# HKUST-Aerial-Robotics/VINS-Mono

Measured on AMD Instinct MI355X. Metric: sliding-window BA solves/sec (Estimator::optimization: 8-iteration dogleg solve + marginalization), higher is better.
Workload: dtype f64; 1 GPU; batch of 256 independent EuRoC-shape windows per step and GPU (K=11 frames, ~150 landmarks, 10 IMU factors, ~600 projection factors, 75-dim marginalization prior, max 8 iterations, MARGIN_OLD marginalization); windows resident in HBM; consecutive steps are issued to 16 HIP streams (independent batches in flight); windows_per_gpu=256, batches_in_flight=16, parallelism=independent batches x1 (no collectives)

## Files before the change

vins-mono_amd/csrc/ba_host.hip:

```cpp
#include "vg_range.h"
#include <hip/hip_runtime.h>
#include <algorithm>
#include <chrono>
#include <cmath>
#include <cstdio>
#include <cstdlib>
#include <cstring>
#include <string>
#include <thread>
#include <vector>
#include "ba_layout.h"
#include "vg_handle.h"
#include "../../include/vinsgpu.h"

struct BaFork { hipStream_t aux; hipEvent_t fork, join; };
extern "C" hipError_t ba_launch_solve(const BaLayout& L, const BaLayout* dL, const BaPtrs& P, int rounds, hipStream_t stream,
                                      hipEvent_t* ev, int* kinds, int* n_launches, const BaFork* fk);
typedef int (*BaAllReduce)(void* user, double* buf, size_t count, void* stream);
extern "C" hipError_t ba_launch_solve_big(const BaLayout& L, const BaLayout* dL, const BaPtrs& P, int rounds, int slack, hipStream_t stream,
                                          BaAllReduce allreduce, void* user, int* hook_rc, hipEvent_t* ev, int* kinds, int* n_launches);
extern "C" hipError_t ba_launch_eval_factors(const BaLayout& L, const BaLayout* dL, const BaPtrs& P, double* proj_r, double* proj_J,
                                            double* imu_r, double* imu_J, double* prior_r, hipStream_t stream);
extern "C" const char* ba_failed_launch();
extern "C" hipError_t ba_prepare_launch();
// ... 252 lines not shown
            if (L.lds_solve_w8 > 160 * 1024) L.sv_w8 = 0;
        }
    }
    if (L.big) {
        const int nt = (L.Rc + 1 + 15) / 16;
        L.nts = nt * (nt + 1) / 2;
        const int ntri = L.Rc * (L.Rc + 1) / 2;
        L.rb1_T = up(ntri + L.Rc, 2);
        L.rb1_scal = L.rb1_T + up((L.Rc + 1) * (L.Rc + 2) / 2, 2);
        L.rb1_len = L.rb1_scal + RB1_NSCAL;
    }
    int o = 0;
    L.io_hdr = o; o += BA_HDR_INTS;
    L.io_lm_start = o; o += L.Lcap;
    L.io_lm_fbeg = o; o += L.Lcap + 8;
    L.io_fac_i = o; o += L.Fcap;
    L.io_fac_j = o; o += L.Fcap;
    L.io_fac_lm = o; o += L.Fcap;
    L.io_fac_oi = o; o += L.Fcap;
    L.io_fac_oj = o; o += L.Fcap;
    L.io_fac_slot = o; o += L.Fcap;
    L.io_pair_ptr = o; o += up(L.Kp * L.Kp + 1, 8);
    L.io_task_list = o; o += up(L.ntask, 8);
    L.io_imu_valid = o; o += up(L.K, 8);
    L.io_pb_kind = o; o += L.NBcap;
    L.io_pb_idx = o; o += L.NBcap;
    L.io_pb_col = o; o += L.NBcap;
    L.io_pb_off = o; o += L.NBcap;
    L.io_pb_x0off = o; o += L.NBcap;
    L.istride = up(o, 8);
    o = 0;
    L.do_pose = o; o += up(7 * L.Kp, 2);
    L.do_sb = o; o += up(9 * L.K, 2);
    L.do_ex = o; o += 8;
    L.do_td = o; o += 2;
    L.do_lam = o; o += L.Lcap;
    L.do_obs = o; o += L.Ocap * BA_OBS_STRIDE;
    L.do_imu = o; o += (L.K - 1) * BA_IMU_STRIDE;
    L.do_par = o; o += P_NPAR;
    L.dstride = up(o, 8);
    L.pld = std::max(up(6 * L.K + 9 * 2 + 6 + 1, 8), L.Ncap);
    L.po_x0 = 0;
    L.po_r0 = 9 * std::max(up(L.K + 4, 8), L.NBcap);
    L.po_J0 = L.po_r0 + L.pld;
    L.pstride = up(L.po_J0 + L.pld * L.pld, 8);
    o = 0;
    L.so_ctl = o; o += C_NCTL;
    L.so_part = o; o += up(L.nbl, 8);
    L.so_x = o; o += 2 * L.nst;
    L.so_lam = o; o += 2 * L.Lcap;
    L.so_imuU = o; o += up((L.K - 1) * 225, 2);
    L.so_Hp = o; o += L.Ncap * L.Ncap;
    L.so_J0t = o; o += L.Ncap * L.Ncap;
    L.so_rec = o; o += L.Fcap * L.REC;
    L.so_sc = o; o += L.Rpad;
    L.so_sl = o; o += L.Lcap;
    L.so_dg = o; o += L.Rpad + L.Lcap;
    L.so_gt = o; o += L.Rpad + L.Lcap;
    L.so_gn = o; o += L.Rpad + L.Lcap;
    L.so_yl = o; o += L.Lcap;
    L.so_lsc = o; o += L.Lcap;
    L.so_xp = 0;
    if (!L.big) { L.so_xp = o; o += up(9 * L.K, 4) * L.ldc; }
    if (L.big) {
        L.so_bigm = o; o += up(bigm_doubles, 8);
        L.so_dgl = o; o += 2 * L.Lcap;
        L.so_gtl = o; o += 2 * L.Lcap;
    }
    {
        int b = 0;
        L.bo_Sp = b; b += up(L.Rc * (L.Rc + 1) / 2, 2);
        L.bo_gp = b; b += L.RcPad;
        L.bo_h = b; b += L.Lcap;
        L.bo_b = b; b += L.Lcap;
        L.bo_Wt = b; b += L.RcPad * L.Lcap;
        L.bo_imuJ = b; b += (L.K - 1) * 512;
        L.bo_pr = b; b += L.Ncap;
        L.bo_gpr = b; b += L.Ncap;
        L.buf_stride = up(b, 8);
    }
    L.so_buf = o; o += 2 * L.buf_stride;
    L.sstride = up(o, 8);
    L.pl_off = (int)((sizeof(BaLayout) + 255) / 256 * 256);
    L.pl_n = L.big ? 0 : L.Rc * (L.Rc + 1) / 2 + L.Rpad + 2 * 81 * L.K;
    o = 0;
    L.oo_pose = o; o += up(7 * L.Kp, 2);
    L.oo_sb = o; o += up(9 * L.K, 2);
    L.oo_ex = o; o += 8;
    L.oo_td = o; o += 2;
    L.oo_lam = o; o += L.Lcap;
    L.oo_sum = o; o += BA_SUM_DOUBLES;
    L.oo_trace = o; o += 5 * VG_MAX_ITERS + 16;
    L.ostride = up(o, 8);
    L.oi_stride = up(4 + VG_MAX_ITERS, 8);
    L.mcap = up(6 * L.K + 9 * 2 + 6 + 1, 8);
    if (L.mcap > 256) { h->err = "kept dimension of the marginalization beyond the kernel's tables"; return VG_ERR_UNSUPPORTED; }
    const int mcap = L.mcap;
    L.mo_J0 = 0;
    L.mo_r0 = mcap * mcap;
    L.mo_x0 = L.mo_r0 + mcap;
    L.mo_stride = up(L.mo_x0 + (L.K + 4) * 9, 8);
    L.mi_stride = up(8 + 2 * (L.K + 4) + 16, 8);
    L.mg_posmax = up(mcap + 15 + L.Lcap, 2);
    {
        const int nstm = up(16 * L.K + 8 + 1, 2);
        L.mg_cs = up(std::max(std::max(2 * mcap, 3 * (L.mg_posmax / 2 + 2)), 2 * (3 * ((mcap + 2) / 2) + 2) + 2), 2);
        L.mg_cs = std::max(L.mg_cs, std::max(up(5 * mcap + 8, 2), up(L.Lcap + 512, 2)));
// ... 1412 lines not shown
```

vins-mono_amd/csrc/ba_pipeline.hip:

```cpp
#include <hip/hip_runtime.h>
#include <vector>
#include <mutex>
#include <cstring>
#include <cstdlib>
#include "ba_layout.h"
#include "ba_factors.h"
#include "../../include/vinsgpu.h"

extern __shared__ __attribute__((aligned(16))) char bp_smem[];

#ifdef BA_SOLVE_W8_TU
#undef BA_PROFILE_DETAIL
#undef BA_DEBUG_DUMP
namespace vg_w8 {
#endif

#define NOINL __device__ __noinline__
#define AS_LDS(p) ((lds_d*)(p))
#define AS_LDS_C(p) ((const lds_d*)(p))
#define AS_GLB(p) ((glb_d*)(p))
#define AS_GLB_C(p) ((const glb_d*)(p))
#define AS_GLB_CI(p) ((const glb_i*)(p))
template <bool BIG> struct MovT { typedef lds_d D; typedef lds_i I; };
template <> struct MovT<true> { typedef glb_d D; typedef glb_i I; };
// ... 274 lines not shown
            for (int r = 0; r < 15; ++r) Uo[r * 15 + i] = (i >= r) ? A[i * 15 + r] : 0.0;
        __syncthreads();
    }
}

NOINL void imu_sqrt_info(const Ctx& c_in, int fbeg, int fend) {
    const Ctx c = c_in;
    const BaLayout L = *c.Lp;
    lds_d* A = AS_LDS(LDSB + c.wave * 256);
    const int nimu = fend < L.K - 1 ? fend : L.K - 1;
    const glb_i* valid = AS_GLB_CI(c.ia + L.io_imu_valid);
    const int li = c.lane < 15 ? c.lane : 14;
    for (int base = fbeg; base < nimu; base += BA_NW) {
        const int f = uni(base + c.wave);
        if (!(f < nimu && valid[f])) continue;
        const glb_d* cov = AS_GLB_C(c.di + L.do_imu + f * BA_IMU_STRIDE + IM_COV);
        double a[15];
#pragma unroll
        for (int k = 0; k < 15; ++k) a[k] = cov[li * 15 + k];
#pragma unroll
        for (int j = 14; j >= 0; --j) {
            const double d = sqrt(readlane_f64(a[j], j));
            a[j] = c.lane < j ? a[j] / d : (c.lane == j ? d : a[j]);
#pragma unroll
            for (int kk = 0; kk < j; ++kk) {
                const double ukj = readlane_f64(a[j], kk);
                a[kk] = (c.lane <= kk) ? a[kk] - a[j] * ukj : a[kk];
            }
        }
        if (c.lane < 15) {
#pragma unroll
            for (int k = 0; k < 15; ++k) A[c.lane * 15 + k] = a[k];
        }
        __builtin_amdgcn_wave_barrier();
        glb_d* Uo = AS_GLB(c.sc + L.so_imuU + f * 225);
        if (c.lane < 15) {
            const int j = c.lane;
            double x[15];
#pragma unroll
            for (int i = 14; i >= 0; --i) {
                double s = (i == j) ? 1.0 : 0.0;
#pragma unroll
                for (int k = 14; k > i; --k) s -= (k <= j) ? A[i * 15 + k] * x[k] : 0.0;
                x[i] = (i <= j) ? s / A[i * 15 + i] : 0.0;
            }
#pragma unroll
            for (int i = 0; i < 15; ++i) Uo[i * 15 + j] = x[i];
        }
        __builtin_amdgcn_wave_barrier();
    }
    __syncthreads();
}

#ifndef BA_SOLVE_W8_TU
extern "C" __global__ __launch_bounds__(BA_NT) void ba_prologue_kernel(const BaLayout* __restrict__ Lp, BaPtrs P) {
    const BaLayout& L = *Lp;
    Ctx c;
    ctx_init(c, Lp, P, blockIdx.x);
    double* x = c.sc + L.so_x;
    DP_DECL;
    const bool all = gridDim.y == 1;
    const int part = blockIdx.y, nI = (L.K - 1 + BA_NW - 1) / BA_NW;
    if (all || part == 0)
    {
        double* out = P.out + (size_t)blockIdx.x * L.ostride;
        int* iout = P.iout + (size_t)blockIdx.x * L.oi_stride;
        int* miout = P.miout + (size_t)blockIdx.x * L.mi_stride;
        for (int k = c.tid; k < L.ostride; k += BA_NT) out[k] = 0.0;
        for (int k = c.tid; k < L.oi_stride; k += BA_NT) iout[k] = 0;
        for (int k = c.tid; k < L.mi_stride; k += BA_NT) miout[k] = 0;
    }
    if (all || part == 0) {
        for (int k = c.tid; k < 7 * L.Kp; k += BA_NT) x[k] = c.di[L.do_pose + k];
        for (int k = c.tid; k < 9 * L.K; k += BA_NT) x[7 * L.Kp + k] = c.di[L.do_sb + k];
        if (c.tid < 7) x[7 * L.Kp + 9 * L.K + c.tid] = c.di[L.do_ex + c.tid];
        if (c.tid == 7) x[7 * L.Kp + 9 * L.K + 7] = c.di[L.do_td];
        for (int k = c.tid; k < c.nL; k += BA_NT) c.sc[L.so_lam + k] = c.di[L.do_lam + k];
        if (c.tid < C_NCTL) {
            double v = 0.0;
            if (c.tid == C_RADIUS) v = 1e4;
            if (c.tid == C_MU || c.tid == C_MUSOLVED) v = 1e-8;
            if (c.tid == C_T0) v = (double)wall_clock64();
            c.sc[L.so_ctl + c.tid] = v;
        }
    }
    DP_ADD(40);
    if (all || (part >= 1 && part <= nI)) {
        const int fbeg = all ? 0 : (part - 1) * BA_NW, fend = all ? L.K - 1 : part * BA_NW;
        if (L.imu_info) imu_sqrt_info_ref(c, fbeg, fend);
        else imu_sqrt_info(c, fbeg, fend);
    }
    DP_ADD(41);
    if (c.nprior && (all || part > nI)) {
        const bool do_copy = all || part == nI + 1, do_prod = all || part == nI + 2;
        const int n = c.nprior;
        const double* J0 = c.pri + L.po_J0;
        double* Hp = c.sc + L.so_Hp;
        if (do_copy) {
            double* J0t = c.sc + L.so_J0t;
            for (int wk = c.tid; wk < n * n; wk += BA_NT) { const int r = wk / n, cc = wk % n; J0t[cc * L.Ncap + r] = J0[r * L.pld + cc]; }
        }
        __syncthreads();
        DP_ADD(42);
        if (!do_prod) {
        } else if ((size_t)n * n * 8 <= (size_t)L.lds_pro) {
            double* J0s = LDSB;
            for (int wk = c.tid; wk < n * n; wk += BA_NT) J0s[wk] = J0[(wk / n) * L.pld + wk % n];
            __syncthreads();
            DP_ADD(43);
            const int T = (n + 15) >> 4, ntile = T * (T + 1) / 2, nks = (n + 3) >> 2;
            const int wave = c.tid >> 6, lane = c.tid & 63, li = lane & 15, lk = lane >> 4;
            for (int t = wave; t < ntile; t += BA_NT / 64) {
                int ta, tb;
                tri_decode(t, ta, tb);
                const int ca = 16 * ta + li, cb = 16 * tb + li;
                double4_t acc = (double4_t){0, 0, 0, 0};
                for (int ks = 0; ks < nks; ++ks) {
                    const int r = 4 * ks + lk;
                    const double av = (r < n && ca < n) ? J0s[r * n + ca] : 0.0;
                    const double bv = (r < n && cb < n) ? J0s[r * n + cb] : 0.0;
                    acc = __builtin_amdgcn_mfma_f64_16x16x4f64(av, bv, acc, 0, 0, 0);
                }
#pragma unroll
                for (int q = 0; q < 4; ++q) {
                    const int a = 16 * ta + lk + 4 * q, bb = 16 * tb + li;
                    if (a < n && bb <= a) {
                        Hp[a * L.Ncap + bb] = acc[q];
                    }
                }
            }
        } else {
            const int ld = L.pld;
            for (int wk = c.tid; wk < n * (n + 1) / 2; wk += BA_NT) {
                int a, bb;
                tri_decode(wk, a, bb);
                double s0 = 0.0, s1 = 0.0;
                int r = 0;
                for (; r + 1 < n; r += 2) { s0 += J0[r * ld + a] * J0[r * ld + bb]; s1 += J0[(r + 1) * ld + a] * J0[(r + 1) * ld + bb]; }
                if (r < n) s0 += J0[r * ld + a] * J0[r * ld + bb];
// ... 230 lines not shown
    double cost = 0.0;
    for (int w = c.tid; w < 4 * L.Ncap; w += BA_NT) {
        const int r = w % L.Ncap, q = w / L.Ncap;
        double sacc = 0.0;
        if (r < n)
            for (int k = q; k < n; k += 4) sacc += Jl[r * ld + k] * dx[k];
        part[w] = sacc;
    }
    __syncthreads();
    lds_d* rl = dx;
    double rv = 0.0;
    const bool own = c.tid < n;
    if (own) rv = r0[c.tid] + ((part[c.tid] + part[L.Ncap + c.tid]) + (part[2 * L.Ncap + c.tid] + part[3 * L.Ncap + c.tid]));
    __syncthreads();
    if (own) { pr[c.tid] = rv; rl[c.tid] = rv; cost += rv * rv; }
    __syncthreads();
    for (int w = c.tid; w < 4 * L.Ncap; w += BA_NT) {
        const int a = w % L.Ncap, q = w / L.Ncap;
        double sacc = 0.0;
        if (a < n)
            for (int k = q; k < n; k += 4) sacc += Jl[k * ld + a] * rl[k];
        part[w] = sacc;
    }
    __syncthreads();
    for (int a = c.tid; a < n; a += BA_NT)
        gpr[a] = (part[a] + part[L.Ncap + a]) + (part[2 * L.Ncap + a] + part[3 * L.Ncap + a]);
    __syncthreads();
    return cost;
}

struct ProjIn {
    double pi[7], pj[7], oi[8], oj[8], ex[8];
    double lam;
    int i, j, l;
};
DEV void proj_fetch(const Ctx& c, int f, const double* x_, const double* lam_, ProjIn& p) {
    const BaLayout& L = *c.Lp;
    const glb_i* ia = AS_GLB_CI(c.ia);
    const glb_d* x = AS_GLB_C(x_);
    const glb_d* obs = AS_GLB_C(c.di + L.do_obs);
    p.i = ia[L.io_fac_i + f];
    p.j = ia[L.io_fac_j + f];
    p.l = ia[L.io_fac_lm + f];
    const int oi = ia[L.io_fac_oi + f], oj = ia[L.io_fac_oj + f];
#pragma unroll
    for (int k = 0; k < 7; ++k) { p.pi[k] = x[7 * p.i + k]; p.pj[k] = x[7 * p.j + k]; }
#pragma unroll
    for (int k = 0; k < 8; ++k) {
        p.oi[k] = obs[oi * BA_OBS_STRIDE + k];
        p.oj[k] = obs[oj * BA_OBS_STRIDE + k];
        p.ex[k] = x[7 * L.Kp + 9 * L.K + k];
    }
    p.lam = AS_GLB_C(lam_)[p.l];
}
DEV void proj_fetch_staged(const Ctx& c, int f, const lds_d* xs, const double* lam_, ProjIn& p) {
    const BaLayout& L = *c.Lp;
    const glb_i* ia = AS_GLB_CI(c.ia);
    const glb_d* obs = AS_GLB_C(c.di + L.do_obs);
    p.i = ia[L.io_fac_i + f];
    p.j = ia[L.io_fac_j + f];
    p.l = ia[L.io_fac_lm + f];
    const int oi = ia[L.io_fac_oi + f], oj = ia[L.io_fac_oj + f];
#pragma unroll
    for (int k = 0; k < 8; ++k) {
        p.oi[k] = obs[oi * BA_OBS_STRIDE + k];
        p.oj[k] = obs[oj * BA_OBS_STRIDE + k];
    }
    p.lam = AS_GLB_C(lam_)[p.l];
#pragma unroll
    for (int k = 0; k < 7; ++k) { p.pi[k] = xs[7 * p.i + k]; p.pj[k] = xs[7 * p.j + k]; }
#pragma unroll
    for (int k = 0; k < 8; ++k) p.ex[k] = xs[7 * L.Kp + 9 * L.K + k];
}
DEV void proj_jac(const Ctx& c, const ProjIn& p, double* r, double* Ji, double* Jj, double* Jex,
                  double* Jl, double* Jtd) {
    const BaLayout& L = *c.Lp;
    if (L.t) {
        if (L.e) proj_eval<true, true, true>(p.pi, p.pj, p.ex, p.lam, p.oi, p.oj, p.ex[7], c.focal, c.tr, c.row, r, Ji, Jj, Jex, Jl, Jtd);
        else proj_eval<true, true, false>(p.pi, p.pj, p.ex, p.lam, p.oi, p.oj, p.ex[7], c.focal, c.tr, c.row, r, Ji, Jj, Jex, Jl, Jtd);
    } else {
        if (L.e) proj_eval<false, true, true>(p.pi, p.pj, p.ex, p.lam, p.oi, p.oj, 0.0, c.focal, c.tr, c.row, r, Ji, Jj, Jex, Jl, Jtd);
        else proj_eval<false, true, false>(p.pi, p.pj, p.ex, p.lam, p.oi, p.oj, 0.0, c.focal, c.tr, c.row, r, Ji, Jj, Jex, Jl, Jtd);
    }
}

NOINL double proj_linearize(const Ctx& c_in, int f, const double* x, const double* lam, double* recs) {
    const Ctx c = c_in;
    const BaLayout L = *c.Lp;
    ProjIn p;
    proj_fetch(c, f, x, lam, p);
    double r[2], Ji[12], Jj[12], Jex[12], Jl[2], Jtd[2];
    proj_jac(c, p, r, Ji, Jj, Jex, Jl, Jtd);
    const double s = r[0] * r[0] + r[1] * r[1];
    const double sq = sqrt(1.0 / (1.0 + s));
    glb_d* rec = AS_GLB(recs) + (size_t)AS_GLB_CI(c.ia)[L.io_fac_slot + f] * L.REC;
#pragma unroll
    for (int k = 0; k < 6; ++k) {
        rec[2 * k] = sq * Ji[k]; rec[2 * k + 1] = sq * Ji[6 + k];
        rec[12 + 2 * k] = sq * Jj[k]; rec[12 + 2 * k + 1] = sq * Jj[6 + k];
    }
    rec[24] = sq * Jl[0]; rec[25] = sq * Jl[1];
    rec[26] = sq * r[0]; rec[27] = sq * r[1];
    if (L.e) {
#pragma unroll
        for (int k = 0; k < 6; ++k) { rec[28 + 2 * k] = sq * Jex[k]; rec[28 + 2 * k + 1] = sq * Jex[6 + k]; }
    }
    if (L.t) { rec[28 + 12 * L.e] = sq * Jtd[0]; rec[29 + 12 * L.e] = sq * Jtd[1]; }
    return log1p(s);
}
NOINL double proj_cost(const Ctx& c_in, int f, const double* x, const double* lam) {
    const Ctx c = c_in;
    const BaLayout L = *c.Lp;
    ProjIn p;
    proj_fetch(c, f, x, lam, p);
    double r[2];
    if (L.t) proj_eval<true, false, false>(p.pi, p.pj, p.ex, p.lam, p.oi, p.oj, p.ex[7], c.focal, c.tr, c.row, r, 0, 0, 0, 0, 0);
    else proj_eval<false, false, false>(p.pi, p.pj, p.ex, p.lam, p.oi, p.oj, 0.0, c.focal, c.tr, c.row, r, 0, 0, 0, 0, 0);
    return log1p(r[0] * r[0] + r[1] * r[1]);
}

#ifndef BA_PROJ_WAVES
#define BA_PROJ_WAVES 1
#endif
#ifndef BA_SOLVE_W8_TU
extern "C" __global__ __launch_bounds__(BA_LIN_NT, BA_PROJ_WAVES) void ba_linearize_proj_kernel(const BaLayout* __restrict__ Lp, BaPtrs P, int cost_only) {
// ... 200 lines not shown
    buf[L.bo_b + l] = b;
    int row = 6 * L.Kp;
    if (L.e | L.t) {
        double wex[6] = {0, 0, 0, 0, 0, 0}, wtd = 0.0;
        const int otd = 28 + 12 * L.e;
        for (int f = fb; f < fe; ++f) {
            const double* rec = recs + (size_t)c.ia[L.io_fac_slot + f] * REC;
            const double l0 = rec[24], l1 = rec[25];
            if (L.e) {
#pragma unroll
                for (int k = 0; k < 6; ++k) wex[k] += rec[28 + 2 * k] * l0 + rec[28 + 2 * k + 1] * l1;
            }
            if (L.t) wtd += rec[otd] * l0 + rec[otd + 1] * l1;
        }
        if (L.e) {
#pragma unroll
            for (int k = 0; k < 6; ++k) Wt[(size_t)(col_ex(L) + k) * ldw] = anchor >= 0 ? wex[k] : 0.0;
            row += 6;
        }
        if (L.t) { Wt[(size_t)col_td(L) * ldw] = anchor >= 0 ? wtd : 0.0; row += 1; }
    }
    if (L.big) { Wt[row * ldw] = b; ++row; }
    for (; row < L.RcPad; ++row) Wt[row * ldw] = 0.0;
}

#ifndef BA_SOLVE_W8_TU
extern "C" __global__ __launch_bounds__(BA_ACC_NT) void ba_accumulate_kernel(const BaLayout* __restrict__ Lp, BaPtrs P) {
    const BaLayout& L = *Lp;
    const int bid = blockIdx.x;
    const int xcd = bid & 7, rest = bid >> 3;
    const int bx = rest % L.nba, w = (rest / L.nba) * 8 + xcd;
    if (w >= L.nwin) return;
    Ctx c;
    ctx_init(c, Lp, P, w);
    const double* ctl = c.sc + L.so_ctl;
    if (ctl[C_DONE] != 0.0) return;
    const int which = ((int)ctl[C_CUR]) ^ (ctl[C_PENDING] != 0.0 ? 1 : 0);
    double* buf = lin_buf(c, which);
    const double* recs = c.sc + L.so_rec;
    __shared__ double part[7 * 36 + 4];
    if (bx < L.Kp) { diag_pose_task(c, bx, recs, buf + L.bo_Sp, buf + L.bo_gp, part); return; }
    const int ng = L.e + L.t;
    if (ng && bx == L.Kp) { global_task(c, recs, buf + L.bo_Sp, buf + L.bo_gp, part); return; }
    const int g = (bx - L.Kp - (ng ? 1 : 0)) * (BA_ACC_NT / 64) + c.wave;
    const int nother = L.ntask - L.Kp - ng * (ng + 1) / 2;
    if (g < nother) owner_task(c, c.ia[L.io_task_list + g], c.lane, recs, buf + L.bo_Sp, buf + L.bo_gp);
    else {
        const int l = (g - nother) * 64 + c.lane;
        if (l < L.Lcap) landmark_task(c, l, recs, buf);
    }
}
#endif

#define LA_NT BA_NT
#define LA_RS 33
#define LA_NPW 6
#define LA_MAXP 13
#define LA_QCAP 80
static_assert(LA_QCAP <= 128, "the pair prefix of ba_linacc_proj_kernel takes two pairs per lane of one wavefront");
#define LA_PAIR 90
DEV int wave_scan_incl(int v) {
    v += __builtin_amdgcn_update_dpp(0, v, 0x111, 0xF, 0xF, true);
    v += __builtin_amdgcn_update_dpp(0, v, 0x112, 0xF, 0xF, true);
    v += __builtin_amdgcn_update_dpp(0, v, 0x114, 0xF, 0xF, true);
    v += __builtin_amdgcn_update_dpp(0, v, 0x118, 0xF, 0xF, true);
    const int r0 = __builtin_amdgcn_readlane(v, 15), r1 = __builtin_amdgcn_readlane(v, 31), r2 = __builtin_amdgcn_readlane(v, 47);
    const int row = (int)(threadIdx.x & 63) >> 4;
    return v + (row > 0 ? r0 : 0) + (row > 1 ? r1 : 0) + (row > 2 ? r2 : 0);
}
DEV int la_pair_q(int i, int j, int Kp) { const int d = j - i; return (d - 1) * Kp - (d - 1) * d / 2 + i; }
__device__ __forceinline__ void linacc_body(const BaLayout* __restrict__ Lp, const BaPtrs& P) {
    const BaLayout L = layout_load(Lp);
    Ctx c;
    ctx_init(c, Lp, P, blockIdx.x);
    const double* ctl = c.sc + L.so_ctl;
    if (ctl[C_DONE] != 0.0) return;
    const int which = uni(((int)ctl[C_CUR]) ^ (ctl[C_PENDING] != 0.0 ? 1 : 0));
    const double* x = c.sc + L.so_x + which * L.nst;
    const double* lam = c.sc + L.so_lam + which * L.Lcap;
    glb_d* buf = AS_GLB(lin_buf(c, which));
    const glb_i* ia = AS_GLB_CI(c.ia);
    lds_d* rec = AS_LDS(LDSB);
    lds_d* Pb = AS_LDS(LDSB + L.la_P);
    lds_i* key = (lds_i*)(LDSB + L.la_key);
    lds_i* lstart = key + L.la_chf;
    lds_i* posx = lstart + 64;
    lds_i* pstart = posx + L.la_chf;
    lds_i* wcnt = pstart + LA_QCAP + 2;
    __shared__ double red[2 * (LA_NT / 64)];
    const int Kp = L.Kp, npair = Kp * (Kp - 1) / 2, chq = L.la_chq;
    const int nL = c.nL;
    DP_DECL;
    {
        double share = 0.0;
        if (c.nprior > 0) {
            if (c.nprior * c.nprior <= 12 * LA_NT && 4 * L.Ncap <= 4 * LA_NT && (c.nprior * (c.nprior + 1) + 2 + 5 * L.Ncap) <= L.la_P)
                share = prior_staged(c, L, x, lin_buf(c, which) + L.bo_pr, lin_buf(c, which) + L.bo_gpr, LDSB);
            else
                share = prior_pass(c, x, lin_buf(c, which) + L.bo_pr, lin_buf(c, which) + L.bo_gpr, LDSB);
        }
        DP_ADD(23);
        share += imu_pass<true>(c, x, lin_buf(c, which) + L.bo_imuJ, 0, L.K - 1);
        const double tot_imu = block_sum(red, LA_NT / 64, c.lane, c.wave, share);
        for (int g = c.tid; g < L.nbl - L.nbf; g += LA_NT) c.sc[L.so_part + L.nbf + g] = g == 0 ? tot_imu : 0.0;
        __syncthreads();
        DP_ADD(22);
    }
    lds_d* xs = AS_LDS(LDSB + L.la_x);
    for (int k = c.tid; k < 7 * L.Kp + 9 * L.K + 8; k += LA_NT) xs[k] = AS_GLB_C(x)[k];
    const int nchunk = nL > 0 ? uni(ia[L.io_lm_fbeg + nL - 1] / chq + 1) : 0;
    for (int t = c.tid; t < nL; t += LA_NT) {
        const int cl = ia[L.io_lm_fbeg + t] / chq;
        if (t == 0 || ia[L.io_lm_fbeg + t - 1] / chq != cl) lstart[cl] = t;
    }
    if (c.tid == 0) lstart[nchunk] = nL;
    for (int e = c.tid; e < npair * LA_PAIR; e += LA_NT) Pb[e] = 0.0;
    const bool pair_wave = c.wave < LA_NPW;
    __syncthreads();
    DP_ADD(24);
    int pidx[4];
#pragma unroll
    for (int reg = 0; reg < 4; ++reg) {
        const int row = (c.lane >> 4) + 4 * reg, col = c.lane & 15;
        int idx = -1;
        if (row < 6) {
            if (col <= row) idx = row * (row + 1) / 2 + col;
            else if (col == 13) idx = 78 + row;
        } else if (row < 12) {
            if (col < 6) idx = 42 + (row - 6) * 6 + col;
            else if (col <= row && col < 12) idx = 21 + (row - 6) * (row - 5) / 2 + (col - 6);
            else if (col == 13) idx = 84 + (row - 6);
        }
        pidx[reg] = idx;
    }
    double cost = 0.0;
    for (int ch = 0; ch < nchunk; ++ch) {
        const int l0 = lstart[ch], l1 = lstart[ch + 1];
        const int f0 = ia[L.io_lm_fbeg + l0], f1 = ia[L.io_lm_fbeg + l1];
        const int nf = uni(f1 - f0);
        if (nf > L.la_chf) __builtin_trap();
        ProjIn pin;
        int q = -1, rank = 0;
        if (c.tid < nf) {
            proj_fetch_staged(c, f0 + c.tid, xs, lam, pin);
            q = la_pair_q(pin.i, pin.j, Kp);
        }
        for (int e = c.tid; e < (LA_NT / 64) * LA_QCAP; e += LA_NT) wcnt[e] = 0;
        __syncthreads();
        DP_ADD(45);
        {
            const unsigned long long act = __ballot(q >= 0);
            unsigned long long same = act;
#pragma unroll
            for (int b = 0; b < 7; ++b) {
                const bool bit = q >= 0 && ((q >> b) & 1);
                const unsigned long long mb = __ballot(bit);
                same &= bit ? mb : ~mb;
            }
            const unsigned long long lt = (1ull << c.lane) - 1ull;
            rank = __popcll(same & lt);
            if (q >= 0 && rank == 0) wcnt[c.wave * LA_QCAP + q] = __popcll(same);
        }
        __syncthreads();
        if (c.wave == 0) {
            int cw0[LA_NT / 64], cw1[LA_NT / 64];
            const int p0 = c.lane, p1 = c.lane + 64;
#pragma unroll
            for (int w = 0; w < LA_NT / 64; ++w) {
                cw0[w] = p0 < npair ? wcnt[w * LA_QCAP + p0] : 0;
                cw1[w] = p1 < npair ? wcnt[w * LA_QCAP + p1] : 0;
            }
            int t0 = 0, t1 = 0;
#pragma unroll
            for (int w = 0; w < LA_NT / 64; ++w) { const int a = cw0[w], b = cw1[w]; cw0[w] = t0; cw1[w] = t1; t0 += a; t1 += b; }
            const int i0 = wave_scan_incl(t0);
            const int tot0 = __builtin_amdgcn_readlane(i0, 63);
            const int i1 = wave_scan_incl(t1) + tot0;
            if (p0 < npair) {
                pstart[p0 + 1] = i0;
#pragma unroll
                for (int w = 0; w < LA_NT / 64; ++w) wcnt[w * LA_QCAP + p0] = i0 - t0 + cw0[w];
            }
            if (p1 < npair) {
                pstart[p1 + 1] = i1;
#pragma unroll
                for (int w = 0; w < LA_NT / 64; ++w) wcnt[w * LA_QCAP + p1] = i1 - t1 + cw1[w];
            }
            if (c.lane == 0) pstart[0] = 0;
        }
        __syncthreads();
        DP_ADD(46);
        if (c.tid < nf) {
            const int pos = wcnt[c.wave * LA_QCAP + q] + rank;
            double r[2], Ji[12], Jj[12], Jl[2];
            proj_eval<false, true, false>(pin.pi, pin.pj, pin.ex, pin.lam, pin.oi, pin.oj, 0.0, c.focal, c.tr, c.row, r, Ji, Jj, nullptr, Jl, nullptr);
            const double s = r[0] * r[0] + r[1] * r[1];
            const double sq = sqrt(1.0 / (1.0 + s));
            lds_d* qr = rec + pos * LA_RS;
#pragma unroll
            for (int k = 0; k < 6; ++k) {
                qr[k] = sq * Ji[k]; qr[16 + k] = sq * Ji[6 + k];
                qr[6 + k] = sq * Jj[k]; qr[22 + k] = sq * Jj[6 + k];
            }
            qr[12] = sq * Jl[0]; qr[28] = sq * Jl[1];
            qr[13] = sq * r[0]; qr[29] = sq * r[1];
            key[c.tid] = pin.i * 16 + pin.j;
            posx[c.tid] = pos;
            cost += log1p(s);
        }
        __syncthreads();
        DP_ADD(25);
        if (pair_wave) {
            double4_t acc[LA_MAXP];
#pragma unroll
            for (int k = 0; k < LA_MAXP; ++k) acc[k] = (double4_t){0, 0, 0, 0};
            const int k4 = c.lane >> 4, col = c.lane & 15;
            const int xo = (k4 & 1) * 16 + col;
            const int hi = k4 >> 1;
            const bool incol = col < 14;
#pragma unroll
            for (int k = 0; k < LA_MAXP; ++k) {
                const int qk = c.wave + LA_NPW * k;
                if (qk >= npair) continue;
                const int pb0 = uni(pstart[qk]), pe0 = uni(pstart[qk + 1]);
                DP_ADD(29);
                for (int e = pb0; e < pe0; e += 4) {
                    const int f0r = e + hi, f1r = e + 2 + hi;
                    const double v0 = (f0r < pe0 && incol) ? rec[f0r * LA_RS + xo] : 0.0;
                    const double v1 = (f1r < pe0 && incol) ? rec[f1r * LA_RS + xo] : 0.0;
                    acc[k] = __builtin_amdgcn_mfma_f64_16x16x4f64(v0, v0, acc[k], 0, 0, 0);
                    if (e + 2 < pe0) acc[k] = __builtin_amdgcn_mfma_f64_16x16x4f64(v1, v1, acc[k], 0, 0, 0);
                }
                DP_ADD(30);
            }
#pragma unroll
            for (int k = 0; k < LA_MAXP; ++k) {
                if (c.wave + LA_NPW * k >= npair) continue;
                lds_d* pb = Pb + (c.wave + LA_NPW * k) * LA_PAIR;
                double old4[4];
#pragma unroll
                for (int reg = 0; reg < 4; ++reg) old4[reg] = (ch > 0 && pidx[reg] >= 0) ? pb[pidx[reg]] : 0.0;
#pragma unroll
                for (int reg = 0; reg < 4; ++reg)
                    if (pidx[reg] >= 0) pb[pidx[reg]] = old4[reg] + acc[k][reg];
            }
            DP_ADD(26);
        } else {
            for (int t = c.tid - LA_NPW * 64; t < l1 - l0; t += LA_NT - LA_NPW * 64) {
                const int l = l0 + t;
                glb_d* Wt = buf + L.bo_Wt + l;
                const size_t ldw = L.Lcap;
                const int fb = ia[L.io_lm_fbeg + l] - f0, fe = ia[L.io_lm_fbeg + l + 1] - f0;
                double h = 0.0, b = 0.0, wi[6] = {0, 0, 0, 0, 0, 0};
                const int anchor = fb < fe ? key[fb] >> 4 : -1;
                int jn = 0;
                for (int f = fb; f < fe; ++f) {
                    const lds_d* q = rec + posx[f] * LA_RS;
                    const int j = key[f] & 15;
                    const double l0v = q[12], l1v = q[28];
                    double v[6];
#pragma unroll
                    for (int k = 0; k < 6; ++k) v[k] = q[6 + k] * l0v + q[22 + k] * l1v;
                    h += l0v * l0v + l1v * l1v;
                    b += l0v * q[13] + l1v * q[29];
#pragma unroll
                    for (int k = 0; k < 6; ++k) wi[k] += q[k] * l0v + q[16 + k] * l1v;
                    for (; jn < j; ++jn) {
                        if (jn == anchor) continue;
#pragma unroll
                        for (int k = 0; k < 6; ++k) Wt[(size_t)(6 * jn + k) * ldw] = 0.0;
                    }
#pragma unroll
                    for (int k = 0; k < 6; ++k) Wt[(size_t)(6 * j + k) * ldw] = v[k];
                    jn = j + 1;
                }
                for (; jn < Kp; ++jn) {
                    if (jn == anchor) continue;
#pragma unroll
                    for (int k = 0; k < 6; ++k) Wt[(size_t)(6 * jn + k) * ldw] = 0.0;
                }
                if (anchor >= 0) {
#pragma unroll
                    for (int k = 0; k < 6; ++k) Wt[(size_t)(6 * anchor + k) * ldw] = wi[k];
                }
                for (int row = 6 * Kp; row < L.RcPad; ++row) Wt[(size_t)row * ldw] = 0.0;
                buf[L.bo_h + l] = h;
// ... 2948 lines not shown
```

vins-mono_amd/csrc/vg_target.h:

```cpp
#pragma once
#include <hip/hip_runtime.h>
#include <stdint.h>

#ifndef VINS_SIMT
typedef __attribute__((address_space(3))) double lds_d;
typedef __attribute__((address_space(3))) int lds_i;
typedef __attribute__((address_space(1))) double glb_d;
typedef __attribute__((address_space(1))) int glb_i;
typedef __attribute__((address_space(1))) uint8_t glb_u8;
typedef __attribute__((address_space(1))) uint32_t glb_u32;
typedef __attribute__((address_space(1))) uint16_t glb_u16;
typedef uint32_t vg_u32_a2 __attribute__((aligned(2)));
typedef __attribute__((address_space(1))) const vg_u32_a2 glb_u32_a2;
#define VG_WAVES_PER_EU(n) __attribute__((amdgpu_waves_per_eu(n, n)))
typedef const __attribute__((address_space(4))) char* vg_kernarg_ptr;
#define BA_WALL_HZ 1e8
#define VG_KEEP_ALIVE(p) asm volatile("" :: "v"(p))
__device__ __forceinline__ int vg_mul24(int a, int b) { return __mul24(a, b); }
__device__ __forceinline__ int uni(int v) { return __builtin_amdgcn_readfirstlane(v); }
__device__ __forceinline__ double uni(double v) {
    return __hiloint2double(__builtin_amdgcn_readfirstlane(__double2hiint(v)), __builtin_amdgcn_readfirstlane(__double2loint(v)));
}
template <typename T>
__device__ __forceinline__ T const_load(const T* p) {
    T v;
    __builtin_memcpy(&v, (const __attribute__((address_space(4))) void*)p, sizeof(T));
    return v;
}
__device__ __forceinline__ uint4 vg_load16_unaligned(const glb_u8* p) {
    typedef unsigned int nv4 __attribute__((ext_vector_type(4), aligned(1)));
    typedef __attribute__((address_space(1))) const nv4 glb_nv4;
    const nv4 t4 = *(glb_nv4*)p;
    uint4 v;
    v.x = t4.x; v.y = t4.y; v.z = t4.z; v.w = t4.w;
    return v;
}
__device__ __forceinline__ int4 vg_load_int4(const void* p) {
    typedef int nv4 __attribute__((ext_vector_type(4)));
    typedef __attribute__((address_space(1))) const nv4 glb_nv4;
    const nv4 t4 = *(glb_nv4*)p;
    int4 v;
    v.x = t4.x; v.y = t4.y; v.z = t4.z; v.w = t4.w;
    return v;
}
template <int Q> __device__ __forceinline__ unsigned vg_byte_pair(unsigned hi, unsigned lo) {
    return __builtin_amdgcn_perm(hi, lo, (unsigned)Q | (0x0Cu << 8) | ((unsigned)(Q + 1) << 16) | (0x0Cu << 24));
}

template <unsigned SEL> __device__ __forceinline__ unsigned vg_perm(unsigned hi, unsigned lo) { return __builtin_amdgcn_perm(hi, lo, SEL); }
typedef unsigned short vg_us2 __attribute__((ext_vector_type(2)));
__device__ __forceinline__ unsigned vg_pk_add(unsigned a, unsigned b) { return __builtin_bit_cast(unsigned, __builtin_bit_cast(vg_us2, a) + __builtin_bit_cast(vg_us2, b)); }
__device__ __forceinline__ unsigned vg_pk_sub(unsigned a, unsigned b) { return __builtin_bit_cast(unsigned, __builtin_bit_cast(vg_us2, a) - __builtin_bit_cast(vg_us2, b)); }
__device__ __forceinline__ unsigned vg_pk_mad(unsigned a, unsigned short k, unsigned c) {
    const vg_us2 kk = {k, k};
    return __builtin_bit_cast(unsigned, __builtin_bit_cast(vg_us2, a) * kk + __builtin_bit_cast(vg_us2, c));
}
__device__ __forceinline__ unsigned vg_pk_shr(unsigned a, unsigned short n) {
    const vg_us2 nn = {n, n};
    return __builtin_bit_cast(unsigned, __builtin_bit_cast(vg_us2, a) >> nn);
}

__device__ __forceinline__ int vg_sdot2(unsigned a, unsigned b, int c) {
    typedef short s2 __attribute__((ext_vector_type(2)));
    return __builtin_amdgcn_sdot2(__builtin_bit_cast(s2, a), __builtin_bit_cast(s2, b), c, false);
}
__device__ __forceinline__ int vg_sdot2_keep(unsigned a, unsigned b, int c) {
    int r;
    asm("v_dot2_i32_i16 %0, %1, %2, %3" : "=v"(r) : "v"(a), "v"(b), "v"(c));
    return r;
}

#else
typedef double lds_d;
typedef int lds_i;
typedef double glb_d;
typedef int glb_i;
typedef uint8_t glb_u8;
typedef uint32_t glb_u32;
typedef uint16_t glb_u16;
typedef uint32_t vg_u32_a2 __attribute__((aligned(2)));
typedef const vg_u32_a2 glb_u32_a2;
#define VG_WAVES_PER_EU(n)
typedef const char* vg_kernarg_ptr;
#define BA_WALL_HZ 1e9
#define VG_KEEP_ALIVE(p) ((void)(p))
inline int vg_mul24(int a, int b) { return a * b; }
inline int uni(int v) { return v; }
inline double uni(double v) { return v; }
template <typename T> inline T const_load(const T* p) { return *p; }
inline uint4 vg_load16_unaligned(const glb_u8* p) { uint4 v; __builtin_memcpy(&v, p, 16); return v; }
inline int4 vg_load_int4(const void* p) { int4 v; __builtin_memcpy(&v, p, 16); return v; }
template <int Q> inline unsigned vg_byte_pair(unsigned hi, unsigned lo) {
    const unsigned long long v = ((unsigned long long)hi << 32) | lo;
    return (unsigned)((v >> (8 * Q)) & 255u) | ((unsigned)((v >> (8 * (Q + 1))) & 255u) << 16);
}
template <unsigned SEL> inline unsigned vg_perm(unsigned hi, unsigned lo) {
    const unsigned long long v = ((unsigned long long)hi << 32) | lo;
    unsigned r = 0;
    for (int i = 0; i < 4; ++i) {
        const unsigned sel = (SEL >> (8 * i)) & 255u;
        if (sel < 8) r |= (unsigned)((v >> (8 * sel)) & 255u) << (8 * i);
        else if (sel != 0x0Cu) { fprintf(stderr, "simt: unmodelled v_perm_b32 selector 0x%x\n", sel); abort(); }
    }
    return r;
}
inline unsigned vg_pk_add(unsigned a, unsigned b) { return ((a + b) & 0xffffu) | (((a >> 16) + (b >> 16)) << 16); }
inline unsigned vg_pk_sub(unsigned a, unsigned b) { return ((a - b) & 0xffffu) | (((a >> 16) - (b >> 16)) << 16); }
inline unsigned vg_pk_mad(unsigned a, unsigned short k, unsigned c) { return (((a & 0xffffu) * k + (c & 0xffffu)) & 0xffffu) | (((a >> 16) * k + (c >> 16)) << 16); }
inline unsigned vg_pk_shr(unsigned a, unsigned short n) { return ((a & 0xffffu) >> n) | (((a >> 16) >> n) << 16); }
inline int vg_sdot2(unsigned a, unsigned b, int c) { return (int)(short)(a & 0xffffu) * (int)(short)(b & 0xffffu) + (int)(short)(a >> 16) * (int)(short)(b >> 16) + c; }
inline int vg_sdot2_keep(unsigned a, unsigned b, int c) { return vg_sdot2(a, b, c); }
#endif
```

Baseline: 184,800 solves/s.

## Precompute projection factor sort table in prologue for fused linacc kernel

The per-iteration chunk sort (ballot-based ranking, prefix scan over camera pairs) and the gather of factor indices and observations are moved out of the fused projection linearization kernel. They are computed once per solve in the prologue and stored in a compact table in scratch. Each linearization iteration then reads the precomputed positions, packed i/j/q, landmark ids and 2-component observations, which removes two block barriers and the sort from the per-iteration path. The pidx computation is also moved next to its use to reduce register pressure. In exchange, the scratch table is larger, the prologue does more work, and the host now rejects configurations with more than 62 chunks.

```diff
diff --git a/vins-mono_amd/csrc/ba_host.hip b/vins-mono_amd/csrc/ba_host.hip
--- a/vins-mono_amd/csrc/ba_host.hip
+++ b/vins-mono_amd/csrc/ba_host.hip
@@ -328,7 +328,16 @@
     L.so_imuU = o; o += up((L.K - 1) * 225, 2);
     L.so_Hp = o; o += L.Ncap * L.Ncap;
     L.so_J0t = o; o += L.Ncap * L.Ncap;
-    L.so_rec = o; o += L.Fcap * L.REC;
+    {
+        int rec = L.Fcap * L.REC;
+        if (L.la_chq > 0 && L.Fcap > 0) {
+            const int nch = (L.Fcap - 1) / L.la_chq + 1;
+            const int tab = 4 * L.Fcap + up(3 * L.Fcap + 2 + 64 + 64 + nch * 82, 2) / 2;
+            if (L.la_on && nch > 62) { h->err = "fused projection kernel: more chunks than its table holds"; return VG_ERR_UNSUPPORTED; }
+            rec = std::max(rec, tab);
+        } else if (L.la_on && L.Fcap > 0) { h->err = "fused projection kernel: no room for its factor table"; return VG_ERR_UNSUPPORTED; }
+        L.so_rec = o; o += rec;
+    }
     L.so_sc = o; o += L.Rpad;
     L.so_sl = o; o += L.Lcap;
     L.so_dg = o; o += L.Rpad + L.Lcap;
diff --git a/vins-mono_amd/csrc/ba_pipeline.hip b/vins-mono_amd/csrc/ba_pipeline.hip
--- a/vins-mono_amd/csrc/ba_pipeline.hip
+++ b/vins-mono_amd/csrc/ba_pipeline.hip
@@ -350,6 +350,130 @@
     __syncthreads();
 }
 
+#define LA_NT BA_NT
+#define LA_RS 33
+#define LA_NPW 6
+#define LA_MAXP 13
+#define LA_QCAP 80
+static_assert(LA_QCAP <= 128, "the pair prefix of ba_linacc_proj_kernel takes two pairs per lane of one wavefront");
+#define LA_PAIR 90
+DEV int wave_scan_incl(int v) {
+    v += __builtin_amdgcn_update_dpp(0, v, 0x111, 0xF, 0xF, true);
+    v += __builtin_amdgcn_update_dpp(0, v, 0x112, 0xF, 0xF, true);
+    v += __builtin_amdgcn_update_dpp(0, v, 0x114, 0xF, 0xF, true);
+    v += __builtin_amdgcn_update_dpp(0, v, 0x118, 0xF, 0xF, true);
+    const int r0 = __builtin_amdgcn_readlane(v, 15), r1 = __builtin_amdgcn_readlane(v, 31), r2 = __builtin_amdgcn_readlane(v, 47);
+    const int row = (int)(threadIdx.x & 63) >> 4;
+    return v + (row > 0 ? r0 : 0) + (row > 1 ? r1 : 0) + (row > 2 ? r2 : 0);
+}
+DEV int la_pair_q(int i, int j, int Kp) { const int d = j - i; return (d - 1) * Kp - (d - 1) * d / 2 + i; }
+#define LA_TAB_PS (LA_QCAP + 2)
+struct LaTab {
+    glb_d* obs;
+    glb_i *ijq, *lm, *pos, *nch, *ls, *fs, *ps;
+};
+DEV LaTab la_table(const BaLayout& L, double* sc) {
+    LaTab t;
+    t.obs = AS_GLB(sc + L.so_rec);
+    t.ijq = (glb_i*)(t.obs + 4 * (size_t)L.Fcap);
+    t.lm = t.ijq + L.Fcap;
+    t.pos = t.lm + L.Fcap;
+    t.nch = t.pos + L.Fcap;
+    t.ls = t.nch + 2;
+    t.fs = t.ls + 64;
+    t.ps = t.fs + 64;
+    return t;
+}
+DEV int la_sort_chunk(int q, int lane, int wave, int npair, lds_i* wcnt, lds_i* pstart) {
+    for (int e = (int)threadIdx.x; e < (LA_NT / 64) * LA_QCAP; e += LA_NT) wcnt[e] = 0;
+    __syncthreads();
+    int rank;
+    {
+        const unsigned long long act = __ballot(q >= 0);
+        unsigned long long same = act;
+#pragma unroll
+        for (int b = 0; b < 7; ++b) {
+            const bool bit = q >= 0 && ((q >> b) & 1);
+            const unsigned long long mb = __ballot(bit);
+            same &= bit ? mb : ~mb;
+        }
+        const unsigned long long lt = (1ull << lane) - 1ull;
+        rank = __popcll(same & lt);
+        if (q >= 0 && rank == 0) wcnt[wave * LA_QCAP + q] = __popcll(same);
+    }
+    __syncthreads();
+    if (wave == 0) {
+        int cw0[LA_NT / 64], cw1[LA_NT / 64];
+        const int p0 = lane, p1 = lane + 64;
+#pragma unroll
+        for (int w = 0; w < LA_NT / 64; ++w) {
+            cw0[w] = p0 < npair ? wcnt[w * LA_QCAP + p0] : 0;
+            cw1[w] = p1 < npair ? wcnt[w * LA_QCAP + p1] : 0;
+        }
+        int t0 = 0, t1 = 0;
+#pragma unroll
+        for (int w = 0; w < LA_NT / 64; ++w) { const int a = cw0[w], b = cw1[w]; cw0[w] = t0; cw1[w] = t1; t0 += a; t1 += b; }
+        const int i0 = wave_scan_incl(t0);
+        const int tot0 = __builtin_amdgcn_readlane(i0, 63);
+        const int i1 = wave_scan_incl(t1) + tot0;
+        if (p0 < npair) {
+            pstart[p0 + 1] = i0;
+#pragma unroll
+            for (int w = 0; w < LA_NT / 64; ++w) wcnt[w * LA_QCAP + p0] = i0 - t0 + cw0[w];
+        }
+        if (p1 < npair) {
+            pstart[p1 + 1] = i1;
+#pragma unroll
+            for (int w = 0; w < LA_NT / 64; ++w) wcnt[w * LA_QCAP + p1] = i1 - t1 + cw1[w];
+        }
+        if (lane == 0) pstart[0] = 0;
+    }
+    __syncthreads();
+    return q >= 0 ? wcnt[wave * LA_QCAP + q] + rank : 0;
+}
+DEV void la_build_table(const Ctx& c, const BaLayout& L) {
+    const glb_i* ia = AS_GLB_CI(c.ia);
+    const glb_d* obs = AS_GLB_C(c.di + L.do_obs);
+    const LaTab T = la_table(L, c.sc);
+    lds_i* lstart = (lds_i*)LDSB;
+    lds_i* pstart = lstart + 64;
+    lds_i* wcnt = pstart + LA_TAB_PS;
+    const int Kp = L.Kp, npair = Kp * (Kp - 1) / 2, chq = L.la_chq;
+    const int nL = c.nL;
+    const int nchunk = nL > 0 ? uni(ia[L.io_lm_fbeg + nL - 1] / chq + 1) : 0;
+    for (int t = c.tid; t < nL; t += LA_NT) {
+        const int cl = ia[L.io_lm_fbeg + t] / chq;
+        if (t == 0 || ia[L.io_lm_fbeg + t - 1] / chq != cl) lstart[cl] = t;
+    }
+    if (c.tid == 0) { lstart[nchunk] = nL; T.nch[0] = nchunk; }
+    __syncthreads();
+    if (c.tid <= nchunk) { T.ls[c.tid] = lstart[c.tid]; T.fs[c.tid] = ia[L.io_lm_fbeg + lstart[c.tid]]; }
+    for (int ch = 0; ch < nchunk; ++ch) {
+        const int l0 = lstart[ch], l1 = lstart[ch + 1];
+        const int f0 = ia[L.io_lm_fbeg + l0], f1 = ia[L.io_lm_fbeg + l1];
+        const int nf = uni(f1 - f0);
+        if (nf > L.la_chf) __builtin_trap();
+        const int f = f0 + c.tid;
+        int i = 0, j = 0, q = -1, oi = 0, oj = 0;
+        if (c.tid < nf) {
+            i = ia[L.io_fac_i + f]; j = ia[L.io_fac_j + f];
+            oi = ia[L.io_fac_oi + f]; oj = ia[L.io_fac_oj + f];
+            T.lm[f] = ia[L.io_fac_lm + f];
+            q = la_pair_q(i, j, Kp);
+        }
+        const int pos = la_sort_chunk(q, c.lane, c.wave, npair, wcnt, pstart);
+        if (c.tid < nf) {
+            T.ijq[f] = i | j << 4 | q << 8;
+            T.pos[f] = pos;
+            const size_t ld = L.Fcap;
+            T.obs[f] = obs[oi * BA_OBS_STRIDE]; T.obs[ld + f] = obs[oi * BA_OBS_STRIDE + 1];
+            T.obs[2 * ld + f] = obs[oj * BA_OBS_STRIDE]; T.obs[3 * ld + f] = obs[oj * BA_OBS_STRIDE + 1];
+        }
+        if (c.tid <= npair) T.ps[ch * LA_TAB_PS + c.tid] = pstart[c.tid];
+        __syncthreads();
+    }
+}
+
 #ifndef BA_SOLVE_W8_TU
 extern "C" __global__ __launch_bounds__(BA_NT) void ba_prologue_kernel(const BaLayout* __restrict__ Lp, BaPtrs P) {
     const BaLayout& L = *Lp;
@@ -383,6 +507,11 @@
         }
     }
     DP_ADD(40);
+    if (L.la_on && (all || part == 0)) {
+        la_build_table(c, L);
+        __syncthreads();
+    }
+    DP_ADD(47);
     if (all || (part >= 1 && part <= nI)) {
         const int fbeg = all ? 0 : (part - 1) * BA_NW, fend = all ? L.K - 1 : part * BA_NW;
         if (L.imu_info) imu_sqrt_info_ref(c, fbeg, fend);
@@ -719,25 +848,6 @@
         p.ex[k] = x[7 * L.Kp + 9 * L.K + k];
     }
     p.lam = AS_GLB_C(lam_)[p.l];
-}
-DEV void proj_fetch_staged(const Ctx& c, int f, const lds_d* xs, const double* lam_, ProjIn& p) {
-    const BaLayout& L = *c.Lp;
-    const glb_i* ia = AS_GLB_CI(c.ia);
-    const glb_d* obs = AS_GLB_C(c.di + L.do_obs);
-    p.i = ia[L.io_fac_i + f];
-    p.j = ia[L.io_fac_j + f];
-    p.l = ia[L.io_fac_lm + f];
-    const int oi = ia[L.io_fac_oi + f], oj = ia[L.io_fac_oj + f];
-#pragma unroll
-    for (int k = 0; k < 8; ++k) {
-        p.oi[k] = obs[oi * BA_OBS_STRIDE + k];
-        p.oj[k] = obs[oj * BA_OBS_STRIDE + k];
-    }
-    p.lam = AS_GLB_C(lam_)[p.l];
-#pragma unroll
-    for (int k = 0; k < 7; ++k) { p.pi[k] = xs[7 * p.i + k]; p.pj[k] = xs[7 * p.j + k]; }
-#pragma unroll
-    for (int k = 0; k < 8; ++k) p.ex[k] = xs[7 * L.Kp + 9 * L.K + k];
 }
 DEV void proj_jac(const Ctx& c, const ProjIn& p, double* r, double* Ji, double* Jj, double* Jex,
                   double* Jl, double* Jtd) {
@@ -1044,23 +1154,15 @@
 }
 #endif
 
-#define LA_NT BA_NT
-#define LA_RS 33
-#define LA_NPW 6
-#define LA_MAXP 13
-#define LA_QCAP 80
-static_assert(LA_QCAP <= 128, "the pair prefix of ba_linacc_proj_kernel takes two pairs per lane of one wavefront");
-#define LA_PAIR 90
-DEV int wave_scan_incl(int v) {
-    v += __builtin_amdgcn_update_dpp(0, v, 0x111, 0xF, 0xF, true);
-    v += __builtin_amdgcn_update_dpp(0, v, 0x112, 0xF, 0xF, true);
-    v += __builtin_amdgcn_update_dpp(0, v, 0x114, 0xF, 0xF, true);
-    v += __builtin_amdgcn_update_dpp(0, v, 0x118, 0xF, 0xF, true);
-    const int r0 = __builtin_amdgcn_readlane(v, 15), r1 = __builtin_amdgcn_readlane(v, 31), r2 = __builtin_amdgcn_readlane(v, 47);
-    const int row = (int)(threadIdx.x & 63) >> 4;
-    return v + (row > 0 ? r0 : 0) + (row > 1 ? r1 : 0) + (row > 2 ? r2 : 0);
-}
-DEV int la_pair_q(int i, int j, int Kp) { const int d = j - i; return (d - 1) * Kp - (d - 1) * d / 2 + i; }
+struct LaIn {
+    double oj[2];
+    double exa[4];
+    double oir[2];
+    double pjr[7], pir[7];
+    double exb[3];
+    double lam;
+    int i, j;
+};
 __device__ __forceinline__ void linacc_body(const BaLayout* __restrict__ Lp, const BaPtrs& P) {
     const BaLayout L = layout_load(Lp);
     Ctx c;
@@ -1078,9 +1180,9 @@
     lds_i* lstart = key + L.la_chf;
     lds_i* posx = lstart + 64;
     lds_i* pstart = posx + L.la_chf;
-    lds_i* wcnt = pstart + LA_QCAP + 2;
+    lds_i* fstart = pstart + LA_QCAP + 2;
     __shared__ double red[2 * (LA_NT / 64)];
-    const int Kp = L.Kp, npair = Kp * (Kp - 1) / 2, chq = L.la_chq;
+    const int Kp = L.Kp, npair = Kp * (Kp - 1) / 2;
     const int nL = c.nL;
     DP_DECL;
     {
@@ -1100,92 +1202,46 @@
     }
     lds_d* xs = AS_LDS(LDSB + L.la_x);
     for (int k = c.tid; k < 7 * L.Kp + 9 * L.K + 8; k += LA_NT) xs[k] = AS_GLB_C(x)[k];
-    const int nchunk = nL > 0 ? uni(ia[L.io_lm_fbeg + nL - 1] / chq + 1) : 0;
-    for (int t = c.tid; t < nL; t += LA_NT) {
-        const int cl = ia[L.io_lm_fbeg + t] / chq;
-        if (t == 0 || ia[L.io_lm_fbeg + t - 1] / chq != cl) lstart[cl] = t;
-    }
-    if (c.tid == 0) lstart[nchunk] = nL;
+    const LaTab T = la_table(L, c.sc);
+    const int nchunk = uni(T.nch[0]);
+    if (c.tid <= nchunk) { lstart[c.tid] = T.ls[c.tid]; fstart[c.tid] = T.fs[c.tid]; }
     for (int e = c.tid; e < npair * LA_PAIR; e += LA_NT) Pb[e] = 0.0;
     const bool pair_wave = c.wave < LA_NPW;
     __syncthreads();
     DP_ADD(24);
-    int pidx[4];
-#pragma unroll
-    for (int reg = 0; reg < 4; ++reg) {
-        const int row = (c.lane >> 4) + 4 * reg, col = c.lane & 15;
-        int idx = -1;
-        if (row < 6) {
-            if (col <= row) idx = row * (row + 1) / 2 + col;
-            else if (col == 13) idx = 78 + row;
-        } else if (row < 12) {
-            if (col < 6) idx = 42 + (row - 6) * 6 + col;
-            else if (col <= row && col < 12) idx = 21 + (row - 6) * (row - 5) / 2 + (col - 6);
-            else if (col == 13) idx = 84 + (row - 6);
-        }
-        pidx[reg] = idx;
-    }
     double cost = 0.0;
     for (int ch = 0; ch < nchunk; ++ch) {
         const int l0 = lstart[ch], l1 = lstart[ch + 1];
-        const int f0 = ia[L.io_lm_fbeg + l0], f1 = ia[L.io_lm_fbeg + l1];
-        const int nf = uni(f1 - f0);
-        if (nf > L.la_chf) __builtin_trap();
-        ProjIn pin;
-        int q = -1, rank = 0;
+        const int f0 = fstart[ch];
+        const int nf = uni(fstart[ch + 1] - f0);
+        LaIn in;
+        int pos = 0;
+        if (c.tid <= npair) pstart[c.tid] = T.ps[ch * LA_TAB_PS + c.tid];
         if (c.tid < nf) {
-            proj_fetch_staged(c, f0 + c.tid, xs, lam, pin);
-            q = la_pair_q(pin.i, pin.j, Kp);
-        }
-        for (int e = c.tid; e < (LA_NT / 64) * LA_QCAP; e += LA_NT) wcnt[e] = 0;
-        __syncthreads();
+            const int f = f0 + c.tid;
+            const size_t ld = L.Fcap;
+            const int ijq = T.ijq[f], l = T.lm[f];
+            pos = T.pos[f];
+            in.i = ijq & 15; in.j = (ijq >> 4) & 15;
+            key[c.tid] = in.i * 16 + in.j;
+            posx[c.tid] = pos;
+            in.oir[1] = T.obs[f]; in.oir[0] = T.obs[ld + f];
+            in.oj[0] = T.obs[2 * ld + f]; in.oj[1] = T.obs[3 * ld + f];
+            in.lam = AS_GLB_C(lam)[l];
+#pragma unroll
+            for (int k = 0; k < 7; ++k) { in.pir[6 - k] = xs[7 * in.i + k]; in.pjr[6 - k] = xs[7 * in.j + k]; }
+#pragma unroll
+            for (int k = 0; k < 7; ++k) (k < 4 ? in.exa[k] : in.exb[k - 4]) = xs[7 * L.Kp + 9 * L.K + k];
+        }
+        __builtin_amdgcn_wave_barrier();
         DP_ADD(45);
-        {
-            const unsigned long long act = __ballot(q >= 0);
-            unsigned long long same = act;
-#pragma unroll
-            for (int b = 0; b < 7; ++b) {
-                const bool bit = q >= 0 && ((q >> b) & 1);
-                const unsigned long long mb = __ballot(bit);
-                same &= bit ? mb : ~mb;
-            }
-            const unsigned long long lt = (1ull << c.lane) - 1ull;
-            rank = __popcll(same & lt);
-            if (q >= 0 && rank == 0) wcnt[c.wave * LA_QCAP + q] = __popcll(same);
-        }
-        __syncthreads();
-        if (c.wave == 0) {
-            int cw0[LA_NT / 64], cw1[LA_NT / 64];
-            const int p0 = c.lane, p1 = c.lane + 64;
-#pragma unroll
-            for (int w = 0; w < LA_NT / 64; ++w) {
-                cw0[w] = p0 < npair ? wcnt[w * LA_QCAP + p0] : 0;
-                cw1[w] = p1 < npair ? wcnt[w * LA_QCAP + p1] : 0;
-            }
-            int t0 = 0, t1 = 0;
-#pragma unroll
-            for (int w = 0; w < LA_NT / 64; ++w) { const int a = cw0[w], b = cw1[w]; cw0[w] = t0; cw1[w] = t1; t0 += a; t1 += b; }
-            const int i0 = wave_scan_incl(t0);
-            const int tot0 = __builtin_amdgcn_readlane(i0, 63);
-            const int i1 = wave_scan_incl(t1) + tot0;
-            if (p0 < npair) {
-                pstart[p0 + 1] = i0;
-#pragma unroll
-                for (int w = 0; w < LA_NT / 64; ++w) wcnt[w * LA_QCAP + p0] = i0 - t0 + cw0[w];
-            }
-            if (p1 < npair) {
-                pstart[p1 + 1] = i1;
-#pragma unroll
-                for (int w = 0; w < LA_NT / 64; ++w) wcnt[w * LA_QCAP + p1] = i1 - t1 + cw1[w];
-            }
-            if (c.lane == 0) pstart[0] = 0;
-        }
-        __syncthreads();
-        DP_ADD(46);
         if (c.tid < nf) {
-            const int pos = wcnt[c.wave * LA_QCAP + q] + rank;
+            double pi[7], pj[7], ex[8], oi[2] = {in.oir[1], in.oir[0]}, oj[2] = {in.oj[0], in.oj[1]};
+#pragma unroll
+            for (int k = 0; k < 7; ++k) { pi[k] = in.pir[6 - k]; pj[k] = in.pjr[6 - k]; ex[k] = k < 4 ? in.exa[k] : in.exb[k - 4]; }
+            ex[7] = 0.0;
             double r[2], Ji[12], Jj[12], Jl[2];
-            proj_eval<false, true, false>(pin.pi, pin.pj, pin.ex, pin.lam, pin.oi, pin.oj, 0.0, c.focal, c.tr, c.row, r, Ji, Jj, nullptr, Jl, nullptr);
+            proj_eval<false, true, false>(pi, pj, ex, in.lam, oi, oj, 0.0, c.focal, c.tr, c.row, r, Ji, Jj, nullptr, Jl, nullptr);
             const double s = r[0] * r[0] + r[1] * r[1];
             const double sq = sqrt(1.0 / (1.0 + s));
             lds_d* qr = rec + pos * LA_RS;
@@ -1196,8 +1252,6 @@
             }
             qr[12] = sq * Jl[0]; qr[28] = sq * Jl[1];
             qr[13] = sq * r[0]; qr[29] = sq * r[1];
-            key[c.tid] = pin.i * 16 + pin.j;
-            posx[c.tid] = pos;
             cost += log1p(s);
         }
         __syncthreads();
@@ -1224,6 +1278,22 @@
                     if (e + 2 < pe0) acc[k] = __builtin_amdgcn_mfma_f64_16x16x4f64(v1, v1, acc[k], 0, 0, 0);
                 }
                 DP_ADD(30);
+            }
+            int pidx[4];
+            const int ln = vg_here(c.lane);
+#pragma unroll
+            for (int reg = 0; reg < 4; ++reg) {
+                const int row = (ln >> 4) + 4 * reg, col = ln & 15;
+                int idx = -1;
+                if (row < 6) {
+                    if (col <= row) idx = row * (row + 1) / 2 + col;
+                    else if (col == 13) idx = 78 + row;
+                } else if (row < 12) {
+                    if (col < 6) idx = 42 + (row - 6) * 6 + col;
+                    else if (col <= row && col < 12) idx = 21 + (row - 6) * (row - 5) / 2 + (col - 6);
+                    else if (col == 13) idx = 84 + (row - 6);
+                }
+                pidx[reg] = idx;
             }
 #pragma unroll
             for (int k = 0; k < LA_MAXP; ++k) {
diff --git a/vins-mono_amd/csrc/vg_target.h b/vins-mono_amd/csrc/vg_target.h
--- a/vins-mono_amd/csrc/vg_target.h
+++ b/vins-mono_amd/csrc/vg_target.h
@@ -16,6 +16,7 @@
 typedef const __attribute__((address_space(4))) char* vg_kernarg_ptr;
 #define BA_WALL_HZ 1e8
 #define VG_KEEP_ALIVE(p) asm volatile("" :: "v"(p))
+__device__ __forceinline__ int vg_here(int v) { asm volatile("" : "+v"(v)); return v; }
 __device__ __forceinline__ int vg_mul24(int a, int b) { return __mul24(a, b); }
 __device__ __forceinline__ int uni(int v) { return __builtin_amdgcn_readfirstlane(v); }
 __device__ __forceinline__ double uni(double v) {
@@ -84,6 +85,7 @@
 typedef const char* vg_kernarg_ptr;
 #define BA_WALL_HZ 1e9
 #define VG_KEEP_ALIVE(p) ((void)(p))
+inline int vg_here(int v) { return v; }
 inline int vg_mul24(int a, int b) { return a * b; }
 inline int uni(int v) { return v; }
 inline double uni(double v) { return v; }
```

Result: no change. 185,300 solves/s, median of 6 (+0.3%).
